# webmproject/sjpeg

Hardware: AMD Instinct MI355X
Metric: Mpixels/s JPEG encode, 4K RGB q=75 YUV420; bit-exact vs ref (higher is better)
Workload: dtype int32/int16 (u8 in); 1 GPU; 64 device-resident 3840x2160 G_struct frames per GPU per step, q=75 YUV420 method 0 (standard Huffman), one complete JPEG per frame; frames_per_gpu=64, width=3840, height=2160, yuv_mode=420, parallelism=frame-sharded x1, no data-path collective, pipelined=True

## Files before the change

### sjpeg_amd/csrc/scan_engine.hip

```cpp
#include <hip/hip_runtime.h>
#include <stdint.h>
#include <stdio.h>
#include <stdlib.h>
#include <string.h>

#include <algorithm>
#include <new>
#include <type_traits>
#include <string>
#include <chrono>
#include <vector>
#include <functional>

#include "sjpeg_hip.h"
#include "jpeg_host.h"
#include "engine.h"

using namespace sjpeg_internal;

namespace {

#include "scan_device.h"
#include "scan_segments.h"
#include "scan_reduce.h"
#include "stitch_kernels.h"


thread_local std::string g_last_error;

}

int sjpeg_internal::set_error(int code, const std::string& msg) {
  g_last_error = msg;
  return code;
}

bool sjpeg_internal::frame_geo(int W, int H, int mode, FrameGeo* g) {
  if (W <= 0 || H <= 0 || W > 65535 || H > 65535) return false;
  switch (mode) {
    case SJPEG_HIP_YUV420: g->bpm = 6; g->px = 16; g->seg_mcus = Geo<SJPEG_HIP_YUV420>::kSegMcus; break;
    case SJPEG_HIP_YUV444: g->bpm = 3; g->px = 8; g->seg_mcus = Geo<SJPEG_HIP_YUV444>::kSegMcus; break;
    case SJPEG_HIP_YUV400: g->bpm = 1; g->px = 8; g->seg_mcus = Geo<SJPEG_HIP_YUV400>::kSegMcus; break;
    default: return false;
  }
  g->mb_w = (W + g->px - 1) / g->px;
  g->mb_h = (H + g->px - 1) / g->px;
  g->n_mcus = g->mb_w * g->mb_h;
  g->nseg = (g->n_mcus + g->seg_mcus - 1) / g->seg_mcus;
  g->slot_words = ((static_cast<uint32_t>(g->seg_mcus) * g->bpm * kMaxBlockBits + 31) / 32 + 2 + 3) & ~3u;
  return true;
}

namespace {

void digest_quant(const sjpeg_hip_scan_tables* t, uint4 (*q)[32]) {
  for (int c = 0; c < 2; ++c) {
    for (int j = 0; j < 64; ++j) {
      uint4& e = q[c][j >> 1];
      const uint32_t iq = t->iquant[c][j], biq = static_cast<uint32_t>(t->bias[c][j]) * iq;
      const uint32_t qv = t->quant[c][j];
      if ((j & 1) == 0) { e.x = iq; e.y = biq; e.w = qv; } else { e.x |= iq << 16; e.z = biq; e.w |= qv << 16; }
    }
  }
}

void digest_tables(const sjpeg_hip_scan_tables* t, DevTables* d) {
  digest_quant(t, d->q);
  memset(d->pad_a, 0, sizeof(d->pad_a));
  memcpy(d->dc, t->dc_codes, sizeof(d->dc));
  memcpy(d->ac, t->ac_codes, sizeof(d->ac));
  memcpy(d->tlen, t->trellis_len, sizeof(d->tlen));
  for (int c = 0; c < 2; ++c) {
    int n_safe = 0;
    for (int n = 1; n <= 10; ++n) {
      const uint32_t len0 = t->ac_codes[c][n] & 0xffu;
      if (len0 + n > 16u) break;
      n_safe = n;
    }
    {
      const uint32_t zrl = t->ac_codes[c][0xf0];
      const uint32_t zl = zrl & 0xffu;
      unsigned long long v = 0;
      d->zrlpat[c][0] = make_uint4(0, 0, 0, 0);
      for (uint32_t k = 1; k <= 3; ++k) {
        v = (v << zl) | (zrl >> 16);
        const unsigned long long left = (zl == 0u) ? 0ull : v << (64u - k * zl);
        d->zrlpat[c][k] = make_uint4(static_cast<uint32_t>(left >> 32), static_cast<uint32_t>(left), k * zl, 0u);
      }
    }
    const uint32_t bad = ~((1u << n_safe) - 1u) & 0x7fffu;
    d->safe_mask[c] = bad | (bad << 16);
    d->eob_zrl[c][0] = t->ac_codes[c][0x00];
    d->eob_zrl[c][1] = t->ac_codes[c][0xf0];
    for (int n = 1; n <= 10; ++n) {
      for (int run = 0; run < 16; ++run) {
        const uint32_t cw = t->ac_codes[c][(run << 4) | n];
        const uint32_t len = cw & 0xffu, code = cw >> 16;
        d->acm[c][run][10 - n] = len == 0u ? 0u : ((code << n) | ((len + n) << 27));
      }
// ... 806 lines not shown
  s.out = static_cast<uint8_t*>(d_out); s.out_stride = out_stride;
  s.sizes = reinterpret_cast<unsigned long long*>(d_sizes);
  s.pack_off = reinterpret_cast<unsigned long long*>(d_pack_off);
  s.seg_nbits64 = nullptr; s.total_bits_out = nullptr; s.subs = 1; s.wide_subs = 0;
  if (static_cast<size_t>(nframes) * g.nseg <= 8192 && (plan.slot_words & 3u) == 0u && plan.slot_words >= 776u) {
    s.subs = (plan.slot_words + kWideSpec * 256u - 1u) / (kWideSpec * 256u);
    s.wide_subs = s.subs > 1u ? 1u : 0u;
    if (!s.wide_subs) s.subs = 1;
  }
  s.hdr_off = multi ? e->hdr_off.p + 2 * static_cast<size_t>(part_first_frame(e)) : nullptr;
  s.seg_first = a.seg_first; s.rst_tail = rst_tail;
  s.frame_flags = e->frame_flags.p;
  static const bool no_fuse_k4 = getenv("SJPEG_HIP_NO_FUSED_K4") != nullptr;
  static const bool no_fuse_big = getenv("SJPEG_HIP_NO_FUSED_BIG") != nullptr;
  const bool fuse_ok = !no_fuse_k4 && !piped && s.pack_off == nullptr && !a.rst && static_cast<size_t>(nframes) * g.nseg <= 8192;
  s.fused_k4 = !fuse_ok ? 0 : max_chunks <= kFusedChunks ? 1 : (nframes == 1 && !no_fuse_big && max_chunks <= kFusedChunksBig) ? 2 : 0;
  static const bool no_fuse_k2 = getenv("SJPEG_HIP_NO_FUSED_K2") != nullptr;
  s.fused_k2 = (!s.fused_k4 || no_fuse_k2 || e->ablate != 0) ? 0 : (s.fused_k4 == 1 && g.nseg <= kFusedSegs) ? 1 : (g.nseg <= kFusedSegsBig && nframes == 1 && !no_fuse_big) ? 2 : 0;
  if (s.fused_k2) {
    a.clear_ff = e->chunk_ff.p; a.clear_n = max_chunks;
    a.clear_per = (max_chunks + static_cast<uint32_t>(g.nseg) - 1u) / static_cast<uint32_t>(g.nseg);
  }

  if ((rc = sync_uploads(e, st))) return rc;
  if (hs != st && (rc = sync_uploads(e, hs))) return rc;
  if (e->timing) HIP_TRY(hipEventRecord(e->ev[0], st));
  if (tables->flags & SJPEG_HIP_QUANT_REPLAY) {
    const int first = e->replay_total > 0 ? e->replay_first : 0;
    const int total = e->replay_total > 0 ? e->replay_total : nframes;
    if (e->replay.p == nullptr || e->replay_w != width || e->replay_h != height || e->replay_mode != yuv_mode ||
        e->replay_nframes != total || first < 0 || first + nframes > total) {
      return fail(SJPEG_HIP_EINVAL, "SJPEG_HIP_QUANT_REPLAY: no kept coefficients of this geometry "
                                    "(run the statistics pass with SJPEG_HIP_QUANT_KEEP first)");
    }
    a.replay = e->replay.p + static_cast<size_t>(first) * g.nseg * kScanThreads * 36;
    rc = launch_scan<kKindEncodeReplay>(yuv_mode, cls, dim3(g.nseg, nframes), st, a);
  } else if (tables->flags & SJPEG_HIP_QUANT_TRELLIS) {
    rc = launch_scan<kKindEncodeTrellis>(yuv_mode, cls, dim3(g.nseg, nframes), st, a);
  } else {
    rc = launch_scan<kKindEncode>(yuv_mode, cls, dim3(g.nseg, nframes), st, a);
  }
  if (rc) return rc;
  dbg_mark("encode: K1 launched");
  if (e->timing) HIP_TRY(hipEventRecord(e->ev[1], st));
  if (piped) {
    HIP_TRY(hipEventRecord(e->k1_done, st));
    dbg_mark("encode: k1_done recorded");
    HIP_TRY(hipStreamWaitEvent(hs, e->k1_done, 0));
    dbg_mark("encode: side waits k1_done");
  }

  if (!s.fused_k2) {
    hipLaunchKernelGGL(scan_seg_offsets<>, dim3(nframes), dim3(kThreads), 0, hs, s);
    HIP_TRY(hipGetLastError());
  }
  dbg_mark("encode: K2 launched");
  uint32_t gx = 4096u / static_cast<uint32_t>(nframes);
  if (gx < 64) gx = 64;
  if (gx > max_chunks) gx = max_chunks;
  if (s.fused_k2 == 2) hipLaunchKernelGGL(place_segments<2>, dim3((g.nseg * s.subs + 3) / 4, nframes), dim3(kThreads), 0, hs, s);
  else if (s.fused_k2) hipLaunchKernelGGL(place_segments<1>, dim3((g.nseg * s.subs + 3) / 4, nframes), dim3(kThreads), 0, hs, s);
  else hipLaunchKernelGGL(place_segments<0>, dim3((g.nseg * s.subs + 3) / 4, nframes), dim3(kThreads), 0, hs, s);
  HIP_TRY(hipGetLastError());
  if (!s.fused_k4) {
    hipLaunchKernelGGL(scan_chunk_offsets<>, dim3(nframes), dim3(kThreads), 0, hs, s);
    HIP_TRY(hipGetLastError());
  }
  e->ctr_clean_at[set] = a.pool_ctr; e->ctr_clean_n[set] = static_cast<size_t>(nframes);
  dbg_mark("encode: K3 K4 launched");
  if (piped) {
    HIP_TRY(hipEventRecord(e->k3_done[set], hs));
    dbg_mark("encode: k3_done recorded");
    e->k3_pending[set] = true;
    e->set = set ^ 1;
  }
  if (s.pack_off != nullptr) {
    hipLaunchKernelGGL(pack_frame_offsets, dim3(1), dim3(kThreads), 0, hs, s);
    HIP_TRY(hipGetLastError());
    hipLaunchKernelGGL(pack_frame_edges, dim3(nframes), dim3(kThreads), 0, hs, s);
    HIP_TRY(hipGetLastError());
  }
  if (s.fused_k4 == 2) hipLaunchKernelGGL(stuff_chunks<2>, dim3(gx, nframes), dim3(kThreads), 0, hs, s);
  else if (s.fused_k4) hipLaunchKernelGGL(stuff_chunks<1>, dim3(gx, nframes), dim3(kThreads), 0, hs, s);
  else hipLaunchKernelGGL(stuff_chunks<0>, dim3(gx, nframes), dim3(kThreads), 0, hs, s);
  HIP_TRY(hipGetLastError());
  dbg_mark("encode: K5 launched");
  if (a.rst && g.nseg - 1 + rst_tail > 0) {
    hipLaunchKernelGGL(patch_restart_markers, dim3((g.nseg - 1 + rst_tail + 3) / 4, nframes), dim3(kThreads), 0, hs, s);
    HIP_TRY(hipGetLastError());
  }
  if (piped) {
    e->side_pending = true;
    e->side_recorded = false;
  }
  if (e->timing) {
    HIP_TRY(hipEventRecord(e->ev[2], hs));
    e->ev_valid = true;
  }
  return 0;
}

static int encode_scan_impl(sjpeg_hip_engine* e, const sjpeg_hip_source* src, int width, int height,
                            int yuv_mode, int nframes, const sjpeg_hip_scan_tables* tables,
                            const void* header, size_t header_size, const size_t* header_offsets,
                            int append_eoi, void* d_out, size_t out_stride, uint64_t* d_sizes,
                            void* stream, const int* seg_range = nullptr, uint64_t* d_pack_off = nullptr) {
  FrameGeo g;
  if (e != nullptr && src != nullptr && nframes > 1 && seg_range == nullptr && d_pack_off == nullptr && d_out != nullptr && d_sizes != nullptr &&
      frame_geo(width, height, yuv_mode, &g)) {
    const SegPlan plan = seg_plan(g, out_stride > 0 ? out_stride : 1);
    const size_t per_frame = ((static_cast<size_t>(g.nseg) * plan.slot_words + plan.pool_words) * (e->pipelined ? 2 : 1) + plan.ubuf_words) * sizeof(uint32_t);
    size_t fit = per_frame == 0 ? static_cast<size_t>(nframes) : e->scratch_limit / per_frame;
    if (fit < 1) fit = 1;
    if (fit < static_cast<size_t>(nframes)) {
      const bool replay = tables != nullptr && (tables->flags & SJPEG_HIP_QUANT_REPLAY) != 0;
      struct Restore { sjpeg_hip_engine* e; int first, total; hipStream_t up; ~Restore() { e->replay_first = first; e->replay_total = total; e->up_stream = up; } } restore{e, e->replay_first, e->replay_total, e->up_stream};
      e->up_stream = nullptr;
      if (replay && e->replay_total <= 0) { e->replay_total = nframes; e->replay_first = 0; }
      const int base_first = e->replay_first;
      for (int f0 = 0; f0 < nframes; f0 += static_cast<int>(fit)) {
        if (replay) e->replay_first = base_first + f0;
        const int nf = nframes - f0 < static_cast<int>(fit) ? nframes - f0 : static_cast<int>(fit);
        sjpeg_hip_source part = *src;
        for (int i = 0; i < 3; ++i) {
          if (part.plane[i] != nullptr) part.plane[i] = static_cast<const uint8_t*>(part.plane[i]) + static_cast<int64_t>(f0) * part.frame_stride[i];
        }
        const bool multi = header_offsets != nullptr;
        const int rc = encode_scan_one(e, &part, width, height, yuv_mode, nf, multi ? tables + f0 : tables, header, header_size,
                                       multi ? header_offsets + f0 : nullptr, append_eoi, static_cast<uint8_t*>(d_out) + static_cast<size_t>(f0) * out_stride,
                                       out_stride, d_sizes + f0, stream);
        if (rc) return rc;
      }
      return 0;
    }
  }
  return encode_scan_one(e, src, width, height, yuv_mode, nframes, tables, header, header_size, header_offsets, append_eoi,
                         d_out, out_stride, d_sizes, stream, seg_range, d_pack_off);
}

int sjpeg_hip_encode_scan_src(sjpeg_hip_engine* e, const sjpeg_hip_source* src, int width, int height,
                              int yuv_mode, int nframes, const sjpeg_hip_scan_tables* tables,
                              const void* header, size_t header_size, int append_eoi, void* d_out,
                              size_t out_stride, uint64_t* d_sizes, void* stream) {
  return encode_scan_impl(e, src, width, height, yuv_mode, nframes, tables, header, header_size, nullptr,
                          append_eoi, d_out, out_stride, d_sizes, stream);
}

int sjpeg_hip_encode_scan_packed_src(sjpeg_hip_engine* e, const sjpeg_hip_source* src, int width, int height,
                                     int yuv_mode, int nframes, const sjpeg_hip_scan_tables* tables,
                                     const void* header, size_t header_size, int append_eoi, void* d_out,
                                     size_t out_stride, uint64_t* d_sizes, uint64_t* d_offsets, void* stream) {
  if (d_offsets == nullptr) return fail(SJPEG_HIP_EINVAL, "sjpeg_hip_encode_scan_packed_src: d_offsets == NULL");
  return encode_scan_impl(e, src, width, height, yuv_mode, nframes, tables, header, header_size, nullptr,
                          append_eoi, d_out, out_stride, d_sizes, stream, nullptr, d_offsets);
}

int sjpeg_hip_encode_intervals_src(sjpeg_hip_engine* e, const sjpeg_hip_source* src, int width, int height,
                                   int yuv_mode, const sjpeg_hip_scan_tables* tables, int seg_begin, int seg_end,
                                   void* d_out, size_t out_cap, uint64_t* d_size, void* stream) {
  if (tables == nullptr || !(tables->flags & SJPEG_HIP_RESTART_MARKERS)) {
    return fail(SJPEG_HIP_EINVAL, "sjpeg_hip_encode_intervals_src needs tables with SJPEG_HIP_RESTART_MARKERS");
  }
  const int range[2] = {seg_begin, seg_end};
  return encode_scan_impl(e, src, width, height, yuv_mode, 1, tables, nullptr, 0, nullptr, 0,
                          d_out, out_cap, d_size, stream, range);
}

// ... 797 lines not shown
  if (rc) return rc;
  if (seg_begin < 0 || seg_end > g.nseg || seg_begin >= seg_end) return fail(SJPEG_HIP_EINVAL, "bad segment range");
  a.rst = 0;
  HIP_TRY(hipMemsetAsync(a.pool_ctr, 0, 2 * sizeof(uint32_t), st));
  e->ctr_clean_at[0] = nullptr;
  const int nloc = seg_end - seg_begin;
  const size_t need = sjpeg_hip_band_bound(width, height, yuv_mode, seg_begin, seg_end);
  if (cap_words < need) {
    return fail(SJPEG_HIP_ECAPACITY, "band buffer of " + std::to_string(cap_words) + " words, need " + std::to_string(need));
  }
  a.nseg = nloc;
  a.seg_first = seg_begin;
  const uint32_t max_chunks = static_cast<uint32_t>((cap_words + kChunkWords - 1) / kChunkWords);
  if ((rc = e->seg_off.ensure(static_cast<size_t>(nloc) + 1))) return rc;
  if ((rc = e->chunk_ff.ensure(max_chunks))) return rc;
  StitchArgs s;
  memset(&s, 0, sizeof(s));
  s.nseg = nloc; s.nframes = 1;
  s.seg_nbits = e->seg_nbits.p; s.seg_off = e->seg_off.p;
  s.seg_words = e->seg_words.p; s.slot_words = plan.slot_words;
  s.pool = a.pool; s.pool_words = plan.pool_words; s.seg_xbase = a.seg_xbase; s.pool_ctr = a.pool_ctr;
  s.ubuf = d_words; s.ubuf_words = cap_words;
  s.chunk_ff = e->chunk_ff.p; s.max_chunks = max_chunks;
  s.total_bits_out = reinterpret_cast<unsigned long long*>(d_nbits);
  s.subs = 1;
  if (tables->flags & SJPEG_HIP_QUANT_TRELLIS) rc = launch_scan<kKindEncodeTrellis>(yuv_mode, cls, dim3(nloc, 1), st, a);
  else rc = launch_scan<kKindEncode>(yuv_mode, cls, dim3(nloc, 1), st, a);
  if (rc) return rc;
  hipLaunchKernelGGL(scan_seg_offsets<>, dim3(1), dim3(kThreads), 0, st, s);
  HIP_TRY(hipGetLastError());
  hipLaunchKernelGGL(place_segments<false>, dim3((nloc + 3) / 4, 1), dim3(kThreads), 0, st, s);
  HIP_TRY(hipGetLastError());
  return 0;
}

int sjpeg_hip_stitch_bands(sjpeg_hip_engine* e, int nbands, const uint32_t* d_words,
                           size_t band_stride_words, const uint64_t* d_nbits, const void* header,
                           size_t header_size, int append_eoi, void* d_out, size_t out_cap,
                           uint64_t* d_size, void* stream) {
  if (e == nullptr || d_words == nullptr || d_nbits == nullptr || d_out == nullptr || d_size == nullptr) {
    return fail(SJPEG_HIP_EINVAL, "null argument");
  }
  if (nbands <= 0 || nbands > 65535) return fail(SJPEG_HIP_EINVAL, "nbands out of range");
  if (band_stride_words < 4 || band_stride_words >= (size_t(1) << 27)) {
    return fail(SJPEG_HIP_EINVAL, "band_stride_words out of range (a band is shorter than 2^32 bits)");
  }
  if (header == nullptr) header_size = 0;
  if (out_cap < header_size + 2 + 64) return fail(SJPEG_HIP_ECAPACITY, "out_cap too small");
  hipStream_t st = static_cast<hipStream_t>(stream);
  HIP_TRY(hipSetDevice(e->device));
  if (int rc0 = order_on_stream(e, st)) return rc0;
  int rc;
  const size_t ubuf_words = (static_cast<size_t>(nbands) * band_stride_words + kChunkWords + 3) & ~size_t(3);
  const uint32_t max_chunks = static_cast<uint32_t>((ubuf_words + kChunkWords - 1) / kChunkWords);
  if ((rc = e->seg_off.ensure(static_cast<size_t>(nbands) + 1))) return rc;
  if ((rc = e->ubuf.ensure(ubuf_words))) return rc;
  if ((rc = e->chunk_ff.ensure(max_chunks))) return rc;
  if ((rc = e->chunk_off.ensure(max_chunks))) return rc;
  if ((rc = e->header.ensure(header_size > 0 ? header_size : 1))) return rc;
  e->header_held_at = nullptr;
  if (header_size > 0) { if (int rcu = upload(e, e->header.p, header, header_size, st)) return rcu; }
  StitchArgs s;
  memset(&s, 0, sizeof(s));
  s.nseg = nbands; s.nframes = 1;
  s.seg_nbits64 = reinterpret_cast<const unsigned long long*>(d_nbits);
  s.seg_off = e->seg_off.p;
  s.seg_words = d_words; s.slot_words = static_cast<uint32_t>(band_stride_words);
  s.ubuf = e->ubuf.p; s.ubuf_words = ubuf_words;
  s.chunk_ff = e->chunk_ff.p; s.chunk_off = e->chunk_off.p; s.max_chunks = max_chunks;
  s.header = e->header.p; s.header_size = static_cast<uint32_t>(header_size);
  s.append_eoi = append_eoi;
  s.out = static_cast<uint8_t*>(d_out); s.out_stride = out_cap;
  s.sizes = reinterpret_cast<unsigned long long*>(d_size);
  const uint32_t per_wave = kSpec * kPlaceLanes;
  s.subs = static_cast<uint32_t>((band_stride_words + per_wave - 1) / per_wave);
  e->last_nseg = nbands; e->last_nframes = 1;
  hipLaunchKernelGGL(scan_seg_offsets<>, dim3(1), dim3(kThreads), 0, st, s);
  HIP_TRY(hipGetLastError());
  const uint32_t units = static_cast<uint32_t>(nbands) * s.subs;
  hipLaunchKernelGGL(place_segments<false>, dim3((units + 3) / 4, 1), dim3(kThreads), 0, st, s);
  HIP_TRY(hipGetLastError());
  hipLaunchKernelGGL(scan_chunk_offsets<>, dim3(1), dim3(kThreads), 0, st, s);
  HIP_TRY(hipGetLastError());
  uint32_t gx = 4096u;
  if (gx > max_chunks) gx = max_chunks;
  hipLaunchKernelGGL(stuff_chunks<false>, dim3(gx, 1), dim3(kThreads), 0, st, s);
  HIP_TRY(hipGetLastError());
  return 0;
}

int sjpeg_hip_adapt_decide(const int64_t* d_sums, const int32_t* d_totlast, int nframes, const uint8_t quant[2][64],
                           int yuv_mode, int qdelta_max_luma, int qdelta_max_chroma, uint8_t* d_quant_out, void* stream) {
  if (d_sums == nullptr || d_totlast == nullptr || quant == nullptr || d_quant_out == nullptr || nframes <= 0 || nframes > 65535) {
    return fail(SJPEG_HIP_EINVAL, "null argument or bad nframes");
  }
  if (qdelta_max_luma < -12 || qdelta_max_luma > 12 || qdelta_max_chroma < -12 || qdelta_max_chroma > 12) {
    return fail(SJPEG_HIP_EINVAL, "qdelta_max outside -12 .. 12");
  }
  return adapt_decide(d_sums, d_totlast, nframes, quant, yuv_mode == SJPEG_HIP_YUV400 ? 1 : 2, qdelta_max_luma, qdelta_max_chroma,
                      d_quant_out, static_cast<hipStream_t>(stream));
}

int sjpeg_hip_adapt_sums(const uint32_t* d_hist, int nframes, const uint8_t quant[2][64],
                         const uint8_t* min_quant, int64_t* d_sums, int32_t* d_totlast, void* stream) {
  if (d_hist == nullptr || quant == nullptr || d_sums == nullptr || d_totlast == nullptr || nframes <= 0 || nframes > 65535) {
    return fail(SJPEG_HIP_EINVAL, "null argument or bad nframes");
  }
  AdaptArgs a;
  a.quant_f = nullptr;
  a.hist = d_hist;
  a.sums = reinterpret_cast<long long*>(d_sums);
  a.totlast = d_totlast;
  memcpy(a.quant, quant, sizeof(a.quant));
  if (min_quant != nullptr) memcpy(a.min_quant, min_quant, sizeof(a.min_quant)); else memset(a.min_quant, 1, sizeof(a.min_quant));
  hipLaunchKernelGGL(adapt_sums_kernel<>, dim3(64, 2, nframes), dim3(64), 0, static_cast<hipStream_t>(stream), a);
  HIP_TRY(hipGetLastError());
  return 0;
}

}
```

### sjpeg_amd/csrc/stitch_kernels.h

```cpp

struct StitchArgs {
  int nseg, nframes;
  const uint32_t* seg_nbits;
  unsigned long long* seg_off;
  const uint32_t* seg_words;
  uint32_t slot_words;
  const uint32_t* pool;
  uint32_t pool_words;
  const uint32_t* seg_xbase;
  const uint32_t* pool_ctr;
  uint32_t* ubuf;
  size_t ubuf_words;
  uint32_t* chunk_ff;
  unsigned long long* chunk_off;
  uint32_t max_chunks;
  const uint8_t* header;
  uint32_t header_size;
  const uint32_t* hdr_off;
  int append_eoi;
  uint8_t* out;
  size_t out_stride;
  unsigned long long* sizes;
  unsigned long long* pack_off = nullptr;
  const unsigned long long* seg_nbits64;
// ... 12 lines not shown

__device__ __forceinline__ StitchArgs ragged_stitch_view(const StitchArgs& in, uint32_t f) {
  const RaggedFrame& d = in.rframes[f];
  StitchArgs v = in;
  v.nseg = d.nseg; v.nframes = 1;
  v.seg_nbits = in.seg_nbits + d.seg_base;
  v.seg_off = in.seg_off + d.seg_base + f;
  v.seg_words = in.seg_words + static_cast<size_t>(d.seg_base) * in.slot_words;
  v.pool = in.pool + d.pool_base; v.pool_words = d.pool_words;
  v.seg_xbase = in.seg_xbase + d.seg_base;
  v.pool_ctr = in.pool_ctr + 2 * f;
  v.ubuf = in.ubuf + d.ubuf_base; v.ubuf_words = d.ubuf_words;
  v.chunk_ff = in.chunk_ff + d.chunk_base; v.chunk_off = in.chunk_off + d.chunk_base; v.max_chunks = d.max_chunks;
  if (in.hdr_off != nullptr) v.hdr_off = in.hdr_off + f;
  v.out = in.out + d.out_offset; v.out_stride = d.out_capacity;
  v.sizes = in.sizes + f;
  v.frame_flags = in.frame_flags + f;
  return v;
}
__device__ __forceinline__ bool frame_overran(const StitchArgs& a, int frame) {
  if (a.pool_ctr == nullptr) return false;
  return a.frame_flags != nullptr ? a.frame_flags[frame] != 0u : a.pool_ctr[2 * frame + 1] != 0u;
}

template <bool RAGGED = false>
__global__ __launch_bounds__(kThreads) void scan_seg_offsets(const StitchArgs a_in) {
  __shared__ uint32_t scratch[16];
  const StitchArgs a = RAGGED ? ragged_stitch_view(a_in, blockIdx.x) : a_in;
  const int frame = RAGGED ? 0 : blockIdx.x;
  const uint32_t* nb = a.seg_nbits + static_cast<size_t>(frame) * a.nseg;
  unsigned long long* off = a.seg_off + static_cast<size_t>(frame) * (a.nseg + 1);
  auto len_of = [&](int i) -> uint32_t {
    return a.seg_nbits64 != nullptr ? static_cast<uint32_t>(a.seg_nbits64[static_cast<size_t>(frame) * a.nseg + i]) : nb[i];
  };
  constexpr int kRun = 8;
  unsigned long long running = 0;
  for (int base = 0; base < a.nseg; base += kThreads * kRun) {
    const int i0 = base + static_cast<int>(threadIdx.x) * kRun;
    uint32_t v[kRun];
    unsigned long long mine = 0;
#pragma unroll
    for (int j = 0; j < kRun; ++j) {
      v[j] = (i0 + j < a.nseg) ? len_of(i0 + j) : 0u;
      mine += v[j];
    }
    unsigned long long at, round_total;
    if (a.seg_nbits64 == nullptr) {
      uint32_t total;
      const uint32_t ex = wg_exclusive_scan<kThreads>(static_cast<uint32_t>(mine), scratch, &total);
      at = running + ex;
      round_total = total;
    } else {
      uint32_t total_lo, total_hi;
      const uint32_t ex_lo = wg_exclusive_scan<kThreads>(static_cast<uint32_t>(mine & 0xffffffu), scratch, &total_lo);
      const uint32_t ex_hi = wg_exclusive_scan<kThreads>(static_cast<uint32_t>(mine >> 24), scratch, &total_hi);
      at = running + ex_lo + (static_cast<unsigned long long>(ex_hi) << 24);
      round_total = total_lo + (static_cast<unsigned long long>(total_hi) << 24);
    }
#pragma unroll
    for (int j = 0; j < kRun; ++j) {
      if (i0 + j < a.nseg) off[i0 + j] = at;
      at += v[j];
    }
    running += round_total;
  }
  if (threadIdx.x == 0) {
    off[a.nseg] = running;
    if (a.total_bits_out != nullptr) a.total_bits_out[frame] = running;
  }
  const unsigned long long U = (running + 7) >> 3;
  unsigned long long nch64 = (U + kChunkBytes - 1) / kChunkBytes;
  if (nch64 > a.max_chunks) nch64 = a.max_chunks;
  const uint32_t nchunks = static_cast<uint32_t>(nch64);
  uint32_t* ff = a.chunk_ff + static_cast<size_t>(frame) * a.max_chunks;
  for (uint32_t i = threadIdx.x; i < nchunks; i += kThreads) ff[i] = 0;
  if (a.frame_flags != nullptr && a.pool_ctr != nullptr && threadIdx.x == 0) {
    a.frame_flags[frame] = a.pool_ctr[2 * frame + 1];
    const_cast<uint32_t*>(a.pool_ctr)[2 * frame] = 0u;
    const_cast<uint32_t*>(a.pool_ctr)[2 * frame + 1] = 0u;
  }
}


__device__ __forceinline__ uint32_t ff_bytes(uint32_t w) {
  return ((w & 0x7f7f7f7fu) + 0x01010101u) & w & 0x80808080u;
}
__device__ __forceinline__ uint32_t count_ff(uint32_t w, int nbytes ) {
  uint32_t n = 0;
#pragma unroll
  for (int b = 0; b < 4; ++b) {
    if (b < nbytes && ((w >> (24 - 8 * b)) & 0xffu) == 0xffu) ++n;
  }
  return n;
}

constexpr int kSpec = 12;
constexpr int kPlaceLanes = 64;
constexpr int kWideSpec = 3;
struct __attribute__((packed, aligned(4))) Words4 { uint32_t w[4]; };
constexpr int kFusedSegs = 2048;
constexpr int kFusedSegsBig = 16384;
template <int FUSED, bool RAGGED = false>
__global__ __launch_bounds__(kThreads) void place_segments(const StitchArgs a_in) {
  __shared__ uint32_t off_lds[FUSED == 1 ? kFusedSegs + 1 : 16];
  __shared__ uint32_t scratch_k2[16];
  const uint32_t rf = RAGGED ? a_in.rmap_place[blockIdx.x] : 0u;
  const uint32_t bx = RAGGED ? blockIdx.x - a_in.rframes[rf].place_base : blockIdx.x;
  const StitchArgs a = RAGGED ? ragged_stitch_view(a_in, rf) : a_in;
  const int frame = RAGGED ? 0 : blockIdx.y;
  const uint32_t* const nb_f = a.seg_nbits + static_cast<size_t>(frame) * a.nseg;
  const int sc_first = static_cast<int>((bx * (kThreads / 64)) / a.subs);
  if (FUSED == 1) {
    const uint32_t* const nb = nb_f;
    constexpr int kRun = kFusedSegs / kThreads;
    const int i0 = static_cast<int>(threadIdx.x) * kRun;
    uint32_t v[kRun], mine = 0;
#pragma unroll
    for (int j = 0; j < kRun; ++j) {
      v[j] = (i0 + j < a.nseg) ? nb[i0 + j] : 0u;
      mine += v[j];
    }
    uint32_t total;
    uint32_t at = wg_exclusive_scan<kThreads>(mine, scratch_k2, &total);
#pragma unroll
    for (int j = 0; j < kRun; ++j) { off_lds[i0 + j] = at; at += v[j]; }
    if (threadIdx.x == 0) {
      off_lds[a.nseg] = total;
      if (bx == 0) {
        a.seg_off[static_cast<size_t>(frame) * (a.nseg + 1) + a.nseg] = total;
        if (a.frame_flags != nullptr && a.pool_ctr != nullptr) a.frame_flags[frame] = a.pool_ctr[2 * frame + 1];
      }
    }
    __syncthreads();
  }
  if (FUSED == 2) {
    uint32_t front = 0, all = 0;
    for (int i = threadIdx.x; i < a.nseg; i += kThreads) {
      const uint32_t v = nb_f[i];
      all += v;
      front += i < sc_first ? v : 0u;
    }
    uint32_t front_total, all_total;
    (void)wg_exclusive_scan<kThreads>(front, scratch_k2, &front_total);
    (void)wg_exclusive_scan<kThreads>(all, scratch_k2, &all_total);
    if (threadIdx.x < 8) {
      uint32_t at = front_total;
      for (int j = 0; j < static_cast<int>(threadIdx.x); ++j) at += sc_first + j < a.nseg ? nb_f[sc_first + j] : 0u;
      off_lds[threadIdx.x] = at;
    }
    if (threadIdx.x == 8) {
      off_lds[8] = all_total;
      if (bx == 0) {
        a.seg_off[static_cast<size_t>(frame) * (a.nseg + 1) + a.nseg] = all_total;
        if (a.frame_flags != nullptr && a.pool_ctr != nullptr) a.frame_flags[frame] = a.pool_ctr[2 * frame + 1];
      }
    }
    __syncthreads();
  }
  const uint32_t unit = bx * (kThreads / kPlaceLanes) + (threadIdx.x >> 6);
  const int sc0 = static_cast<int>(unit / a.subs);
  const uint32_t ibase = (unit % a.subs) * (a.wide_subs ? kWideSpec * 256u : kSpec * kPlaceLanes);
  if (sc0 >= a.nseg) return;
  const unsigned long long* const off_g = a.seg_off + static_cast<size_t>(frame) * (a.nseg + 1);
  auto off = [&](int i) -> unsigned long long {
    if (FUSED == 1) return off_lds[i];
    if (FUSED == 2) {
      if (i >= a.nseg) return off_lds[8];
      if (i - sc_first < 8) return off_lds[i - sc_first];
      unsigned long long at = off_lds[7];
      for (int j = sc_first + 7; j < i; ++j) at += nb_f[j];
      return at;
    }
    return off_g[i];
  };
  const uint32_t* segw = a.seg_words + static_cast<size_t>(frame) * a.nseg * a.slot_words;
  const uint32_t* src = segw + static_cast<size_t>(sc0) * a.slot_words;
  const bool wide = (a.subs == 1u || a.wide_subs) && (a.slot_words & 3u) == 0u && a.slot_words >= 776u;
// ... 434 lines not shown
      *valid = (U - byte0 >= 16) ? 16 : static_cast<int>(U - byte0);
      if (byte0 + 16 < U) *behind = ub[w0 + 4];
    }
  };
  uint4 q_next;
  uint32_t behind_next;
  int valid_next;
  unsigned long long off_next;
  auto gdx_of = [&]() -> uint32_t { return RAGGED ? a_in.rframes[rf].stuff_wgs : gridDim.x; };
  fetch(bx, &q_next, &behind_next, &valid_next, &off_next);
  for (uint32_t chunk = bx; chunk < nchunks; chunk += gdx_of()) {
    const uint4 q = q_next;
    const uint32_t behind = behind_next;
    const int valid = valid_next;
    const unsigned long long chunk_off = FUSED == 2 ? static_cast<unsigned long long>(big_off) : off_next;
    fetch(chunk + gdx_of(), &q_next, &behind_next, &valid_next, &off_next);
    if (FUSED == 2 && chunk + gdx_of() < nchunks) {
      uint32_t mine = 0, step;
      for (uint32_t i = chunk + threadIdx.x; i < chunk + gdx_of(); i += kThreads) mine += ff_f[i];
      (void)wg_exclusive_scan<kThreads>(mine, scratch, &step);
      big_off += step;
    }
    const uint32_t w[4] = {q.x, q.y, q.z, q.w};
    uint32_t ffs = 0;
    if (valid == 16) {
#pragma unroll
      for (int j = 0; j < 4; ++j) ffs += __popc(ff_bytes(w[j]));
    } else {
#pragma unroll
      for (int j = 0; j < 4; ++j) ffs += count_ff(w[j], valid - 4 * j);
    }
    uint32_t total_ff;
    const uint32_t ex = wg_exclusive_scan<kThreads>(ffs, scratch, &total_ff);
    uint8_t* const dchunk = dst0 + static_cast<unsigned long long>(chunk) * kChunkBytes + chunk_off;
    const uint32_t mis = static_cast<uint32_t>(reinterpret_cast<uintptr_t>(dchunk) & 15u);
    const uint32_t o = mis + threadIdx.x * 16 + ex;
    const uint32_t n0 = behind >> 24, n1 = (behind >> 16) & 0xffu, n2 = (behind >> 8) & 0xffu;
    const bool behind_plain = (ff_bytes(behind) & 0x80808000u) == 0u;
    if (valid == 16 && ffs == 0u && behind_plain) {
      const uint32_t m[5] = {__builtin_bswap32(w[0]), __builtin_bswap32(w[1]), __builtin_bswap32(w[2]),
                             __builtin_bswap32(w[3]), __builtin_bswap32(behind)};
      const uint32_t up = (0u - o) & 3u;
      uint32_t d[4];
#pragma unroll
      for (int k = 0; k < 4; ++k) d[k] = __builtin_amdgcn_alignbyte(m[k + 1], m[k], up);
      uint32_t* const sp = reinterpret_cast<uint32_t*>(stage + o + up);
      sp[0] = d[0]; sp[1] = d[1]; sp[2] = d[2]; sp[3] = d[3];
      if (threadIdx.x == 0) {
        for (uint32_t j = 0; j < up; ++j) stage[o + j] = static_cast<uint8_t>(m[0] >> (8 * j));
      }
    } else {
      uint8_t* sp = stage + o;
#pragma unroll
      for (int j = 0; j < 16; ++j) {
        if (j < valid) {
          const uint8_t b = static_cast<uint8_t>(w[j >> 2] >> (24 - 8 * (j & 3)));
          *sp++ = b;
          if (b == 0xff) *sp++ = 0x00;
        }
      }
      sp[0] = static_cast<uint8_t>(n0);
      sp[1] = static_cast<uint8_t>(n0 == 0xffu ? 0u : n1);
      sp[2] = static_cast<uint8_t>(n0 == 0xffu ? n1 : (n1 == 0xffu ? 0u : n2));
    }
    __syncthreads();
    const unsigned long long rest = U - static_cast<unsigned long long>(chunk) * kChunkBytes;
    const uint32_t nbytes = static_cast<uint32_t>(rest < kChunkBytes ? rest : kChunkBytes) + total_ff;
    uint8_t* const dalign = dchunk - mis;
    const uint32_t lo = mis, hi = mis + nbytes;
    const uint32_t first_full = (lo + 15u) & ~15u, last_full = hi & ~15u;
    if (first_full <= last_full) {
      for (uint32_t i = first_full / 16 + threadIdx.x; i < last_full / 16; i += kThreads) {
        reinterpret_cast<uint4*>(dalign)[i] = reinterpret_cast<const uint4*>(stage)[i];
      }
      if (threadIdx.x < first_full - lo) dalign[lo + threadIdx.x] = stage[lo + threadIdx.x];
      if (threadIdx.x < hi - last_full) dalign[last_full + threadIdx.x] = stage[last_full + threadIdx.x];
    } else {
      if (threadIdx.x < nbytes) dalign[lo + threadIdx.x] = stage[lo + threadIdx.x];
    }
    __syncthreads();
  }
}



__global__ __launch_bounds__(kThreads) void patch_restart_markers(const StitchArgs a) {
  const int frame = blockIdx.y;
  const int s = static_cast<int>(blockIdx.x * (kThreads / 64) + (threadIdx.x >> 6));
  const int lane = threadIdx.x & 63;
  if (s >= a.nseg - (a.rst_tail ? 0 : 1) || a.sizes[frame] == 0) return;
  const unsigned long long end_bits = a.seg_off[static_cast<size_t>(frame) * (a.nseg + 1) + s + 1];
  const unsigned long long p = (end_bits >> 3) - 2;
  const unsigned long long chunk = p / kChunkBytes, cstart = chunk * kChunkBytes;
  const uint32_t* ub = a.ubuf + static_cast<size_t>(frame) * a.ubuf_words;
  uint32_t ffs = 0;
  for (unsigned long long b = cstart + 4ull * lane; b < p; b += 256) {
    const unsigned long long left = p - b;
    ffs += count_ff(ub[b >> 2], left >= 4 ? 4 : static_cast<int>(left));
  }
  for (int d = 32; d > 0; d >>= 1) ffs += __shfl_down(ffs, d, 64);
  if (lane == 0) {
    const uint32_t hsize = a.hdr_off ? a.hdr_off[frame + 1] - a.hdr_off[frame] : a.header_size;
    uint8_t* dst = frame_out(a, frame) + hsize + p +
                   a.chunk_off[static_cast<size_t>(frame) * a.max_chunks + chunk] + ffs;
    dst[0] = 0xff;
    dst[1] = static_cast<uint8_t>(0xd0 + ((s + a.seg_first) & 7));
  }
}

__global__ __launch_bounds__(kThreads) void counted_bits_ragged(const StitchArgs a_in, unsigned long long* bits) {
  __shared__ unsigned long long red[kThreads / 64];
  const StitchArgs a = ragged_stitch_view(a_in, blockIdx.x);
  const unsigned long long T = a.seg_off[a.nseg];
  const unsigned long long U = (T + 7) >> 3;
  const bool fits = ((U + 3) >> 2) + 1 <= a.ubuf_words && !frame_overran(a, 0);
  unsigned long long nch = (U + kChunkBytes - 1) / kChunkBytes;
  if (nch > a.max_chunks) nch = a.max_chunks;
  unsigned long long ff = 0;
  if (fits) {
    for (unsigned long long i = threadIdx.x; i < nch; i += kThreads) ff += a.chunk_ff[i];
  }
  for (int d = 32; d > 0; d >>= 1) ff += __shfl_xor(ff, d, 64);
  if ((threadIdx.x & 63) == 0) red[threadIdx.x >> 6] = ff;
  __syncthreads();
  if (threadIdx.x != 0) return;
  if (!fits) { bits[blockIdx.x] = ~0ull; return; }
  ff = red[0] + red[1] + red[2] + red[3];
  if ((T & 7) != 0) {
    const uint32_t w = a.ubuf[(U - 1) >> 2];
    if (((w >> (24 - 8 * ((U - 1) & 3))) & 0xffu) == 0xffu) --ff;
  }
  bits[blockIdx.x] = T + 8 * ff;
}
```

Before: 593,500 Mpixels/s.

## Replace block-per-chunk byte stuffing with wave-per-chunk register-based stuffing kernel

```diff
diff --git a/sjpeg_amd/csrc/scan_engine.hip b/sjpeg_amd/csrc/scan_engine.hip
--- a/sjpeg_amd/csrc/scan_engine.hip
+++ b/sjpeg_amd/csrc/scan_engine.hip
@@ -15,6 +15,7 @@
 #include "sjpeg_hip.h"
 #include "jpeg_host.h"
 #include "engine.h"
+#include "stuff_wave_body.h"
 
 using namespace sjpeg_internal;
 
@@ -987,7 +988,7 @@
   }
   if (s.fused_k4 == 2) hipLaunchKernelGGL(stuff_chunks<2>, dim3(gx, nframes), dim3(kThreads), 0, hs, s);
   else if (s.fused_k4) hipLaunchKernelGGL(stuff_chunks<1>, dim3(gx, nframes), dim3(kThreads), 0, hs, s);
-  else hipLaunchKernelGGL(stuff_chunks<0>, dim3(gx, nframes), dim3(kThreads), 0, hs, s);
+  else hipLaunchKernelGGL(stuff_chunks_wave, dim3((max_chunks + 3u) / 4u, nframes), dim3(kThreads), 0, hs, s);
   HIP_TRY(hipGetLastError());
   dbg_mark("encode: K5 launched");
   if (a.rst && g.nseg - 1 + rst_tail > 0) {
@@ -1951,9 +1952,7 @@
   HIP_TRY(hipGetLastError());
   hipLaunchKernelGGL(scan_chunk_offsets<>, dim3(1), dim3(kThreads), 0, st, s);
   HIP_TRY(hipGetLastError());
-  uint32_t gx = 4096u;
-  if (gx > max_chunks) gx = max_chunks;
-  hipLaunchKernelGGL(stuff_chunks<false>, dim3(gx, 1), dim3(kThreads), 0, st, s);
+  hipLaunchKernelGGL(stuff_chunks_wave, dim3((max_chunks + 3u) / 4u, 1), dim3(kThreads), 0, st, s);
   HIP_TRY(hipGetLastError());
   return 0;
 }
diff --git a/sjpeg_amd/csrc/stitch_kernels.h b/sjpeg_amd/csrc/stitch_kernels.h
--- a/sjpeg_amd/csrc/stitch_kernels.h
+++ b/sjpeg_amd/csrc/stitch_kernels.h
@@ -118,17 +118,6 @@
 }
 
 
-__device__ __forceinline__ uint32_t ff_bytes(uint32_t w) {
-  return ((w & 0x7f7f7f7fu) + 0x01010101u) & w & 0x80808080u;
-}
-__device__ __forceinline__ uint32_t count_ff(uint32_t w, int nbytes ) {
-  uint32_t n = 0;
-#pragma unroll
-  for (int b = 0; b < 4; ++b) {
-    if (b < nbytes && ((w >> (24 - 8 * b)) & 0xffu) == 0xffu) ++n;
-  }
-  return n;
-}
 
 constexpr int kSpec = 12;
 constexpr int kPlaceLanes = 64;
@@ -729,6 +718,40 @@
   }
 }
 
+__global__ __launch_bounds__(kThreads, 8) void stuff_chunks_wave(const StitchArgs a) {
+  const int frame = blockIdx.y;
+  const uint32_t wave = static_cast<uint32_t>(__builtin_amdgcn_readfirstlane(static_cast<int>(threadIdx.x >> 6)));
+  const uint32_t lane = threadIdx.x & 63u;
+  const uint32_t chunk = blockIdx.x * (kThreads / 64) + wave;
+  const unsigned long long T = a.seg_off[static_cast<size_t>(frame) * (a.nseg + 1) + a.nseg];
+  const unsigned long long U = (T + 7) >> 3;
+  const unsigned long long nchunks = (U + kChunkBytes - 1) / kChunkBytes;
+  if (chunk >= nchunks || a.sizes[frame] == 0) return;
+  const uint32_t* const ub = a.ubuf + static_cast<size_t>(frame) * a.ubuf_words + static_cast<size_t>(chunk) * kChunkWords;
+  const unsigned long long left = U - static_cast<unsigned long long>(chunk) * kChunkBytes;
+  const uint32_t rest = left < kChunkBytes ? static_cast<uint32_t>(left) : static_cast<uint32_t>(kChunkBytes);
+  const uint32_t hsize = a.hdr_off ? a.hdr_off[frame + 1] - a.hdr_off[frame] : a.header_size;
+  uint8_t* const base = frame_out(a, frame) + hsize + static_cast<unsigned long long>(chunk) * kChunkBytes +
+                        a.chunk_off[static_cast<size_t>(frame) * a.max_chunks + chunk];
+  constexpr uint32_t kSub = kChunkBytes / 4;
+  uint4 q[4];
+  int valid[4];
+#pragma unroll
+  for (int k = 0; k < 4; ++k) {
+    const uint32_t at = k * kSub + 16u * lane;
+    valid[k] = stuff_valid(rest, at);
+    q[k] = *reinterpret_cast<const uint4*>(ub + ((valid[k] != 0 ? at : 0u) >> 2));
+  }
+  uint32_t running = 0;
+#pragma unroll
+  for (int k = 0; k < 4; ++k) {
+    const StuffLane l = stuff_lane(q[k].x, q[k].y, q[k].z, q[k].w);
+    const uint32_t count = stuff_count(l, valid[k]);
+    const uint32_t incl = wave_inclusive_scan(count);
+    stuff_store(base, k * kSub + 16u * lane + running + (incl - count), l, valid[k], count);
+    running += static_cast<uint32_t>(__builtin_amdgcn_readlane(static_cast<int>(incl), 63));
+  }
+}
 
 
 __global__ __launch_bounds__(kThreads) void patch_restart_markers(const StitchArgs a) {
diff --git a/sjpeg_amd/csrc/stuff_wave_body.h b/sjpeg_amd/csrc/stuff_wave_body.h
--- /dev/null
+++ b/sjpeg_amd/csrc/stuff_wave_body.h
@@ -0,0 +1,138 @@
+#ifndef SJPEG_AMD_STUFF_WAVE_BODY_H_
+#define SJPEG_AMD_STUFF_WAVE_BODY_H_
+
+#include <stdint.h>
+
+#if defined(__HIPCC__)
+#define SJPEG_STUFF_HD __host__ __device__ __forceinline__
+#else
+#define SJPEG_STUFF_HD inline
+#endif
+#ifndef SJPEG_STUFF_STORE
+#define SJPEG_STUFF_STORE(p, n) ((void)0)
+#endif
+
+namespace sjpeg_internal {
+
+SJPEG_STUFF_HD uint32_t ff_bytes(uint32_t w) {
+  return ((w & 0x7f7f7f7fu) + 0x01010101u) & w & 0x80808080u;
+}
+SJPEG_STUFF_HD uint32_t count_ff(uint32_t w, int nbytes ) {
+  uint32_t n = 0;
+#pragma unroll
+  for (int b = 0; b < 4; ++b) {
+    if (b < nbytes && ((w >> (24 - 8 * b)) & 0xffu) == 0xffu) ++n;
+  }
+  return n;
+}
+
+struct __attribute__((packed, aligned(1))) StuffBytes16 { uint32_t v[4]; };
+struct __attribute__((packed, aligned(1))) StuffBytes8 { uint32_t v[2]; };
+struct __attribute__((packed, aligned(1))) StuffBytes4 { uint32_t v; };
+struct __attribute__((packed, aligned(1))) StuffBytes2 { uint16_t v; };
+
+SJPEG_STUFF_HD int stuff_valid(uint32_t rest, uint32_t at) {
+  const int v = static_cast<int>(rest) - static_cast<int>(at);
+  return v < 0 ? 0 : v > 16 ? 16 : v;
+}
+
+struct StuffLane { uint32_t w[4], d[4], t[4]; };
+SJPEG_STUFF_HD StuffLane stuff_lane(uint32_t w0, uint32_t w1, uint32_t w2, uint32_t w3) {
+  StuffLane l;
+  l.w[0] = w0; l.w[1] = w1; l.w[2] = w2; l.w[3] = w3;
+#pragma unroll
+  for (int j = 0; j < 4; ++j) {
+    l.d[j] = __builtin_bswap32(l.w[j]);
+    l.t[j] = ff_bytes(l.d[j]);
+  }
+  return l;
+}
+
+SJPEG_STUFF_HD uint32_t stuff_count(const StuffLane& l, int valid) {
+  uint32_t n = 0;
+  if (valid == 16) {
+#pragma unroll
+    for (int j = 0; j < 4; ++j) n += static_cast<uint32_t>(__builtin_popcount(l.t[j]));
+  } else {
+#pragma unroll
+    for (int j = 0; j < 4; ++j) n += count_ff(l.w[j], valid - 4 * j);
+  }
+  return n;
+}
+
+SJPEG_STUFF_HD uint32_t stuff_shr(uint32_t hi, uint32_t lo, uint32_t s) {
+  return static_cast<uint32_t>(((static_cast<uint64_t>(hi) << 32) | lo) >> s);
+}
+
+SJPEG_STUFF_HD void stuff_store(uint8_t* base, uint32_t off, const StuffLane& l, int valid, uint32_t count) {
+  uint32_t d0 = l.d[0], d1 = l.d[1], d2 = l.d[2], d3 = l.d[3];
+  if (valid == 16 && count == 0u) {
+    SJPEG_STUFF_STORE(base + off, 16);
+    *reinterpret_cast<StuffBytes16*>(base + off) = StuffBytes16{{d0, d1, d2, d3}};
+    return;
+  }
+  if (valid == 0) return;
+  if (valid == 16 && count == 1u) {
+    const unsigned __int128 t = static_cast<unsigned __int128>(l.t[0]) | static_cast<unsigned __int128>(l.t[1]) << 32 |
+                                static_cast<unsigned __int128>(l.t[2]) << 64 | static_cast<unsigned __int128>(l.t[3]) << 96;
+    const unsigned __int128 low128 = t | (t - 1);
+    uint32_t stay[4], move[4];
+    const uint32_t d[4] = {d0, d1, d2, d3};
+#pragma unroll
+    for (int k = 0; k < 4; ++k) {
+      const uint32_t low = static_cast<uint32_t>(low128 >> (32 * k));
+      stay[k] = d[k] & low;
+      move[k] = d[k] & ~low;
+    }
+    SJPEG_STUFF_STORE(base + off, 16);
+    *reinterpret_cast<StuffBytes16*>(base + off) =
+        StuffBytes16{{stay[0] | move[0] << 8, stay[1] | stuff_shr(move[1], move[0], 24), stay[2] | stuff_shr(move[2], move[1], 24),
+                      stay[3] | stuff_shr(move[3], move[2], 24)}};
+    SJPEG_STUFF_STORE(base + (off + 16u), 1);
+    base[off + 16u] = static_cast<uint8_t>(move[3] >> 24);
+    return;
+  }
+  uint32_t mask = (l.t[0] * 0x00204081u) >> 28 | ((l.t[1] * 0x00204081u) >> 28) << 4 |
+                  ((l.t[2] * 0x00204081u) >> 28) << 8 | ((l.t[3] * 0x00204081u) >> 28) << 12;
+  mask &= 0xffffu >> (16 - valid);
+  uint32_t pos = 0;
+  for (;;) {
+    const uint32_t end = mask != 0u ? static_cast<uint32_t>(__builtin_ctz(mask)) + 1u : static_cast<uint32_t>(valid);
+    const uint32_t n = end - pos;
+    if (n & 16u) {
+      SJPEG_STUFF_STORE(base + off, 16);
+      *reinterpret_cast<StuffBytes16*>(base + off) = StuffBytes16{{d0, d1, d2, d3}};
+    }
+    if (n & 8u) {
+      SJPEG_STUFF_STORE(base + off, 8);
+      *reinterpret_cast<StuffBytes8*>(base + off) = StuffBytes8{{d0, d1}};
+      d0 = d2; d1 = d3;
+    }
+    if (n & 4u) {
+      SJPEG_STUFF_STORE(base + (off + (n & 8u)), 4);
+      *reinterpret_cast<StuffBytes4*>(base + (off + (n & 8u))) = StuffBytes4{d0};
+      d0 = d1; d1 = d2; d2 = d3;
+    }
+    if (n & 2u) {
+      SJPEG_STUFF_STORE(base + (off + (n & 12u)), 2);
+      *reinterpret_cast<StuffBytes2*>(base + (off + (n & 12u))) = StuffBytes2{static_cast<uint16_t>(d0)};
+    }
+    if (n & 1u) {
+      SJPEG_STUFF_STORE(base + (off + (n & 14u)), 1);
+      base[off + (n & 14u)] = static_cast<uint8_t>(d0 >> (8u * (n & 2u)));
+    }
+    const uint32_t r = 8u * (n & 3u);
+    d0 = stuff_shr(d1, d0, r); d1 = stuff_shr(d2, d1, r); d2 = stuff_shr(d3, d2, r); d3 >>= r;
+    off += n;
+    if (mask == 0u) break;
+    SJPEG_STUFF_STORE(base + off, 1);
+    base[off] = 0;
+    off += 1u;
+    mask &= mask - 1u;
+    pos = end;
+  }
+}
+
+}
+
+#endif
```

After: 608,800 Mpixels/s, median of 6. 1.03x the previous value.
